# NethermindEth/stark-rings

Measured on AMD Instinct MI355X. Metric: ring-muls/sec (Goldilocks, deg 2^16, batch 2^14), higher is better.
Workload: dtype u64; 1 GPU; goldilocks_d65536_b16384; ring=goldilocks, degree=65536, batch_per_gpu=16384, global_batch=16384, layout=ark-ff Montgomery u64 limbs, in place (a *= b), b read-only, variant=mul, parallelism=batch-sharded x1, twiddle broadcast only

## Files before the change

include/stark_rings_hip.h:

```cpp
#ifndef STARK_RINGS_HIP_H
#define STARK_RINGS_HIP_H

#include <stddef.h>
#include <stdint.h>

#ifdef __cplusplus
extern "C" {
#endif

enum sr_ring {
    SR_RING_GOLDILOCKS_POW2 = 0,
    SR_RING_BABYBEAR_POW2 = 1,
    SR_RING_STARK_POW2 = 2,
    SR_RING_GOLDILOCKS_24 = 3,
    SR_RING_BABYBEAR_72 = 4,
    SR_RING_FROG_16 = 5
};

enum sr_status {
    SR_OK = 0,
    SR_E_INVALID = 1,
    SR_E_NO_DEVICE = 2,
    SR_E_HIP = 3,
    SR_E_ALLOC = 4,
    SR_E_UNSUPPORTED = 5
};

typedef struct sr_ctx sr_ctx;

int sr_ctx_create(int ring, int log2_degree, int device, sr_ctx **out);
enum sr_plan_flags {
    SR_PLAN_GENERIC_KERNELS = 1u << 0,
    SR_PLAN_GL_NO_COLS256 = 1u << 1,
    SR_PLAN_RT_NO_COLS256 = 1u << 2,
    SR_PLAN_GL_REGTILE = 1u << 3,
    SR_PLAN_STARK_NO_LAZY = 1u << 4,
    SR_PLAN_STARK_GENERIC_ON_LAZY = 1u << 5,
    SR_PLAN_NO_HOST_PIN = 1u << 6,
    SR_PLAN_GL_PLAIN_COLS = 1u << 7,
    SR_PLAN_GL_SPLIT_ROWS = 1u << 8
};
typedef struct sr_plan {
    uint32_t flags;
    int32_t log_tile;
    int32_t stark_whole_max;
    uint32_t chunk_polys;
    uint64_t scratch_limit_bytes;
    uint32_t host_chunk_mb;
    uint32_t lanes;
} sr_plan;
int sr_ctx_create_ex(int ring, int log2_degree, int device, const sr_plan *plan, sr_ctx **out);
int sr_ctx_reserve_scratch(sr_ctx *ctx, size_t batch);
int sr_ctx_plan_in_use(sr_ctx *ctx, sr_plan *plan, double probe_ms[2], size_t *probe_elems);
int sr_ctx_destroy(sr_ctx *ctx);
int sr_ctx_degree(const sr_ctx *ctx, size_t *degree);
int sr_ctx_limbs(const sr_ctx *ctx, int *limbs);
int sr_ctx_twiddle_block(sr_ctx *ctx, void **dev_ptr, size_t *bytes);
int sr_ctx_twiddles_updated(sr_ctx *ctx);
int sr_ctx_create_group(int ring, int log2_degree, const int *device_ids, int n, const sr_plan *plan, sr_ctx **out);
int sr_shard_range(size_t batch, int n, int i, size_t *first, size_t *count);

int sr_ntt_fwd_batch(sr_ctx *ctx, uint64_t *data, size_t batch);
int sr_ntt_inv_batch(sr_ctx *ctx, uint64_t *data, size_t batch);
int sr_pointwise_mul_batch(sr_ctx *ctx, uint64_t *lhs_inout, const uint64_t *rhs, size_t batch);
int sr_add_batch(sr_ctx *ctx, uint64_t *lhs_inout, const uint64_t *rhs, size_t batch);
int sr_sub_batch(sr_ctx *ctx, uint64_t *lhs_inout, const uint64_t *rhs, size_t batch);
int sr_neg_batch(sr_ctx *ctx, uint64_t *data, size_t batch);
int sr_scale_batch(sr_ctx *ctx, uint64_t *data, const uint64_t *scalar, size_t batch);
int sr_add_scalar_batch(sr_ctx *ctx, uint64_t *data, const uint64_t *scalar, int ntt_form, size_t batch);
int sr_mul_elem_batch(sr_ctx *ctx, uint64_t *data_inout, const uint64_t *elem, size_t batch);
int sr_sum_batch(sr_ctx *ctx, uint64_t *out, const uint64_t *in, size_t n);
int sr_product_batch(sr_ctx *ctx, uint64_t *out, const uint64_t *in_ntt, size_t n);
int sr_mul_elem_add_batch(sr_ctx *ctx, uint64_t *acc_inout, const uint64_t *x, const uint64_t *r, size_t batch);
int sr_ring_mul_batch(sr_ctx *ctx, uint64_t *out, const uint64_t *a, const uint64_t *b, size_t batch);
int sr_reduce_batch(sr_ctx *ctx, const uint64_t *in, size_t in_len_per_elem, uint64_t *out, size_t batch);

int sr_ntt_fwd_batch_dev(sr_ctx *ctx, uint64_t *d_data, size_t batch, void *stream);
int sr_ntt_inv_batch_dev(sr_ctx *ctx, uint64_t *d_data, size_t batch, void *stream);
int sr_pointwise_mul_batch_dev(sr_ctx *ctx, uint64_t *d_lhs_inout, const uint64_t *d_rhs, size_t batch, void *stream);
int sr_add_batch_dev(sr_ctx *ctx, uint64_t *d_lhs_inout, const uint64_t *d_rhs, size_t batch, void *stream);
int sr_sub_batch_dev(sr_ctx *ctx, uint64_t *d_lhs_inout, const uint64_t *d_rhs, size_t batch, void *stream);
int sr_neg_batch_dev(sr_ctx *ctx, uint64_t *d_data, size_t batch, void *stream);
int sr_scale_batch_dev(sr_ctx *ctx, uint64_t *d_data, const uint64_t *host_scalar, size_t batch, void *stream);
int sr_add_scalar_batch_dev(sr_ctx *ctx, uint64_t *d_data, const uint64_t *host_scalar, int ntt_form, size_t batch, void *stream);
int sr_mul_elem_batch_dev(sr_ctx *ctx, uint64_t *d_data_inout, const uint64_t *d_elem, size_t batch, void *stream);
int sr_sum_batch_dev(sr_ctx *ctx, uint64_t *d_out, const uint64_t *d_in, size_t n, void *stream);
int sr_product_batch_dev(sr_ctx *ctx, uint64_t *d_out, const uint64_t *d_in_ntt, size_t n, void *stream);
int sr_mul_elem_add_batch_dev(sr_ctx *ctx, uint64_t *d_acc_inout, const uint64_t *d_x, const uint64_t *d_r, size_t batch, void *stream);
enum { SR_MLE_LEADING = 0, SR_MLE_TRAILING = 1 };
int sr_mle_plan(int ring, int log2_degree, size_t num_vars, size_t n_fixed, int order, size_t *work_elems, int *launches);
int sr_mle_fix_variables_dev(sr_ctx *ctx, uint64_t *d_out, const uint64_t *d_evals, size_t n_evals, size_t num_vars, const uint64_t *d_point,
                             size_t n_fixed, int order, uint64_t *d_work, size_t work_elems, void *stream);
int sr_mle_fix_variables(sr_ctx *ctx, uint64_t *out, const uint64_t *evals, size_t n_evals, size_t num_vars, const uint64_t *point,
// ... 79 lines not shown
```

stark_rings_amd/_lib.py:

```python
import ctypes
import os

HERE = os.path.dirname(os.path.abspath(__file__))
LIB_PATH = os.environ.get("SR_LIB_PATH") or os.path.join(HERE, "libstarkrings_hip.so")

u64p = ctypes.POINTER(ctypes.c_uint64)
_c = ctypes

SYMBOLS = {
    "sr_ctx_create": (_c.c_int, [_c.c_int, _c.c_int, _c.c_int, _c.POINTER(_c.c_void_p)]),
    "sr_ctx_create_ex": (_c.c_int, [_c.c_int, _c.c_int, _c.c_int, _c.c_void_p, _c.POINTER(_c.c_void_p)]),
    "sr_ctx_create_group": (_c.c_int, [_c.c_int, _c.c_int, _c.POINTER(_c.c_int), _c.c_int, _c.c_void_p, _c.POINTER(_c.c_void_p)]),
    "sr_shard_range": (_c.c_int, [_c.c_size_t, _c.c_int, _c.c_int, _c.POINTER(_c.c_size_t), _c.POINTER(_c.c_size_t)]),
    "sr_ctx_reserve_scratch": (_c.c_int, [_c.c_void_p, _c.c_size_t]),
    "sr_ctx_plan_in_use": (_c.c_int, [_c.c_void_p, _c.c_void_p, _c.POINTER(_c.c_double), _c.POINTER(_c.c_size_t)]),
    "sr_ctx_destroy": (_c.c_int, [_c.c_void_p]),
    "sr_ctx_degree": (_c.c_int, [_c.c_void_p, _c.POINTER(_c.c_size_t)]),
    "sr_ctx_limbs": (_c.c_int, [_c.c_void_p, _c.POINTER(_c.c_int)]),
    "sr_ctx_twiddle_block": (_c.c_int, [_c.c_void_p, _c.POINTER(_c.c_void_p), _c.POINTER(_c.c_size_t)]),
    "sr_ctx_twiddles_updated": (_c.c_int, [_c.c_void_p]),
    "sr_ntt_fwd_batch": (_c.c_int, [_c.c_void_p, u64p, _c.c_size_t]),
    "sr_ntt_inv_batch": (_c.c_int, [_c.c_void_p, u64p, _c.c_size_t]),
    "sr_pointwise_mul_batch": (_c.c_int, [_c.c_void_p, u64p, u64p, _c.c_size_t]),
    "sr_add_batch": (_c.c_int, [_c.c_void_p, u64p, u64p, _c.c_size_t]),
# ... 36 lines not shown
    "sr_matmul_ntt": (_c.c_int, [_c.c_void_p] * 4 + [_c.c_size_t] * 3),
    "sr_decompose_balanced_batch_dev": (_c.c_int, [_c.c_void_p] * 3 + [_c.c_uint64, _c.c_size_t, _c.c_size_t, _c.c_void_p]),
    "sr_decompose_overflow_count": (_c.c_int, [_c.c_void_p, _c.POINTER(_c.c_ulonglong), _c.c_void_p]),
    "sr_recompose_batch_dev": (_c.c_int, [_c.c_void_p] * 3 + [_c.c_uint64, _c.c_size_t, _c.c_size_t, _c.c_void_p]),
    "sr_decompose_balanced_batch": (_c.c_int, [_c.c_void_p] * 3 + [_c.c_uint64, _c.c_size_t, _c.c_size_t]),
    "sr_recompose_batch": (_c.c_int, [_c.c_void_p] * 3 + [_c.c_uint64, _c.c_size_t, _c.c_size_t]),
    "sr_decompose_balanced_batch_wide_dev": (_c.c_int, [_c.c_void_p] * 3 + [_c.c_uint64, _c.c_uint64, _c.c_size_t, _c.c_size_t, _c.c_void_p]),
    "sr_recompose_batch_wide_dev": (_c.c_int, [_c.c_void_p] * 3 + [_c.c_uint64, _c.c_uint64, _c.c_size_t, _c.c_size_t, _c.c_void_p]),
    "sr_decompose_balanced_batch_wide": (_c.c_int, [_c.c_void_p] * 3 + [_c.c_uint64, _c.c_uint64, _c.c_size_t, _c.c_size_t]),
    "sr_recompose_batch_wide": (_c.c_int, [_c.c_void_p] * 3 + [_c.c_uint64, _c.c_uint64, _c.c_size_t, _c.c_size_t]),
    "sr_wire_coeff_bytes": (_c.c_size_t, [_c.c_void_p]),
    "sr_serialize_batch_dev": (_c.c_int, [_c.c_void_p] * 4 + [_c.c_size_t, _c.c_void_p]),
    "sr_deserialize_batch_dev": (_c.c_int, [_c.c_void_p] * 4 + [_c.c_size_t, _c.c_void_p]),
    "sr_wire_invalid_count": (_c.c_int, [_c.c_void_p, _c.POINTER(_c.c_ulonglong), _c.c_void_p]),
    "sr_serialize_batch": (_c.c_int, [_c.c_void_p] * 3 + [_c.c_size_t]),
    "sr_deserialize_batch": (_c.c_int, [_c.c_void_p] * 3 + [_c.c_size_t]),
    "sr_rot_batch_dev": (_c.c_int, [_c.c_void_p] * 3 + [_c.c_size_t, _c.c_void_p]),
    "sr_rot_batch": (_c.c_int, [_c.c_void_p, u64p, _c.c_size_t]),
    "sr_ring_mul_batch_dev": (_c.c_int, [_c.c_void_p, _c.c_void_p, _c.c_void_p, _c.c_void_p, _c.c_size_t, _c.c_void_p]),
    "sr_ring_mul_ntt_rhs_batch": (_c.c_int, [_c.c_void_p, u64p, u64p, u64p, _c.c_size_t]),
    "sr_ring_mul_ntt_rhs_batch_dev": (_c.c_int, [_c.c_void_p, _c.c_void_p, _c.c_void_p, _c.c_void_p, _c.c_size_t, _c.c_void_p]),
    "sr_pack32_batch_dev": (_c.c_int, [_c.c_void_p, _c.c_void_p, _c.c_void_p, _c.c_size_t, _c.c_void_p]),
    "sr_unpack32_batch_dev": (_c.c_int, [_c.c_void_p, _c.c_void_p, _c.c_void_p, _c.c_size_t, _c.c_void_p]),
    "sr_ntt_fwd_packed32_batch_dev": (_c.c_int, [_c.c_void_p, _c.c_void_p, _c.c_size_t, _c.c_void_p]),
    "sr_ntt_inv_packed32_batch_dev": (_c.c_int, [_c.c_void_p, _c.c_void_p, _c.c_size_t, _c.c_void_p]),
    "sr_ring_mul_packed32_batch_dev": (_c.c_int, [_c.c_void_p, _c.c_void_p, _c.c_void_p, _c.c_void_p, _c.c_size_t, _c.c_void_p]),
    "sr_pointwise_mul_packed32_batch_dev": (_c.c_int, [_c.c_void_p, _c.c_void_p, _c.c_void_p, _c.c_size_t, _c.c_void_p]),
    "sr_add_packed32_batch_dev": (_c.c_int, [_c.c_void_p, _c.c_void_p, _c.c_void_p, _c.c_size_t, _c.c_void_p]),
    "sr_sub_packed32_batch_dev": (_c.c_int, [_c.c_void_p, _c.c_void_p, _c.c_void_p, _c.c_size_t, _c.c_void_p]),
    "sr_reduce_batch_dev": (_c.c_int, [_c.c_void_p, _c.c_void_p, _c.c_size_t, _c.c_void_p, _c.c_size_t, _c.c_void_p]),
    "sr_fill_uniform_dev": (_c.c_int, [_c.c_void_p, _c.c_uint64, _c.c_uint64, _c.c_size_t, _c.c_void_p, _c.c_void_p]),
    "sr_count_noncanonical_dev": (_c.c_int, [_c.c_void_p, _c.c_void_p, _c.c_size_t, _c.POINTER(_c.c_uint64), _c.c_void_p]),
    "sr_ctx_profile_enable": (_c.c_int, [_c.c_void_p, _c.c_int]),
    "sr_ctx_profile_read": (_c.c_int, [_c.c_void_p, _c.POINTER(_c.c_double), _c.POINTER(_c.c_uint64)]),
    "sr_ctx_profile_read_sampled": (_c.c_int, [_c.c_void_p, _c.POINTER(_c.c_double), _c.POINTER(_c.c_uint64), _c.POINTER(_c.c_uint64)]),
    "sr_selftest_field_op": (_c.c_int, [_c.c_int, _c.c_int, u64p, u64p, u64p]),
    "sr_selftest_rep_counters": (_c.c_int, [u64p, _c.c_int]),
    "sr_last_error_string": (_c.c_char_p, []),
    "sr_version": (_c.c_char_p, []),
}



class Plan(ctypes.Structure):
    _fields_ = [("flags", _c.c_uint32), ("log_tile", _c.c_int32), ("stark_whole_max", _c.c_int32), ("chunk_polys", _c.c_uint32),
                ("scratch_limit_bytes", _c.c_uint64), ("host_chunk_mb", _c.c_uint32), ("lanes", _c.c_uint32)]


PLAN_GENERIC_KERNELS, PLAN_GL_NO_COLS256, PLAN_RT_NO_COLS256 = 1, 2, 4
PLAN_GL_REGTILE, PLAN_STARK_NO_LAZY, PLAN_STARK_GENERIC_ON_LAZY = 8, 16, 32
PLAN_NO_HOST_PIN = 64
PLAN_GL_PLAIN_COLS = 128
PLAN_GL_SPLIT_ROWS = 256


def plan_from_env(ring=None):
    e = os.environ
    f = 0
    if (ring in (None, 0) and e.get("SR_GOLDILOCKS_GENERIC") == "1") or (ring in (None, 1) and e.get("SR_BABYBEAR_GENERIC") == "1"):
        f |= PLAN_GENERIC_KERNELS
    if e.get("SR_GL_COLS256") == "0":
        f |= PLAN_GL_NO_COLS256
    if e.get("SR_RT_COLS256") == "0":
        f |= PLAN_RT_NO_COLS256
    if e.get("SR_GOLDILOCKS_REGTILE") == "1":
        f |= PLAN_GL_REGTILE
    if e.get("SR_STARK_LAZY") == "0":
        f |= PLAN_STARK_NO_LAZY
    if e.get("SR_STARK_TUNED") == "0":
        f |= PLAN_STARK_GENERIC_ON_LAZY
    if e.get("SR_HOST_PIN") == "0":
        f |= PLAN_NO_HOST_PIN
    if e.get("SR_GL_KEEP_COLS") == "0":
        f |= PLAN_GL_PLAIN_COLS
    if e.get("SR_GL_SPLIT_ROWS") == "1":
        f |= PLAN_GL_SPLIT_ROWS
    p = Plan()
    p.flags = f
    p.log_tile = int(e.get("SR_LOG_TILE", "0") or 0)
    p.stark_whole_max = int(e.get("SR_ST_WHOLE_MAX", "0") or 0)
    p.chunk_polys = int(e.get("SR_CHUNK_POLYS", "0") or 0)
    p.scratch_limit_bytes = int(e.get("SR_SCRATCH_LIMIT_MB", "0") or 0) << 20
    p.host_chunk_mb = int(e.get("SR_HOST_CHUNK_MB", "0") or 0)
    p.lanes = int(e.get("SR_LANES", "0") or 0)
    return p


_lib = None


class BackendMissing(RuntimeError):
    pass


def load():
    global _lib
    if _lib is None:
        if not os.path.exists(LIB_PATH):
            raise BackendMissing(
                "%s not found: run `python -c 'import __graft_entry__ as g; g.build()'` "
                "(hipcc --offload-arch=gfx950).  There is no CPU fallback." % LIB_PATH
            )
        try:
            import torch
        except Exception:
            pass
        lib = ctypes.CDLL(LIB_PATH)
        for name, (res, args) in SYMBOLS.items():
            fn = getattr(lib, name)
            fn.restype = res
            fn.argtypes = args
        _lib = lib
    return _lib


def last_error():
    return load().sr_last_error_string().decode()
```

stark_rings_amd/csrc/capi.hip:

```cpp
#include "../../include/stark_rings_hip.h"

#include <hip/hip_runtime.h>

#include <cstdio>
#include <cstring>
#include <condition_variable>
#include <functional>
#include <initializer_list>
#include <mutex>
#include <string>
#include <thread>
#include <type_traits>
#include <vector>

#include "fields.hpp"
#include "ntt_generic.hpp"
#include "ntt_goldilocks.hpp"
#include "ntt_regtile.hpp"
#include "small_rings.hpp"
#include "small_linalg.hpp"
#include "decompose.hpp"
#include "wire.hpp"
#include "frog_ring.hpp"
#include "ntt_stark.hpp"
// ... 248 lines not shown
    const int k = c->k;
    if (k > F::kTwoAdicity - 1) return fail(SR_E_INVALID, "log2_degree exceeds the field's 2-adicity");
    c->log_tile = default_log_tile<F>();
    if (c->plan.log_tile >= 8 && c->plan.log_tile <= 12) c->log_tile = c->plan.log_tile;
    if (k > 2 * c->log_tile && !stark_tuned) return fail(SR_E_INVALID, "log2_degree too large for the two-level kernels");
    const size_t d = c->degree;
    size_t extra = 0;
    if constexpr (std::is_same<F, sr::Goldilocks>::value) extra = sr::gl_fast_extra_bytes(k);
    c->table_bytes = 2 * d * sizeof(E) + extra;
    HIP_TRY(hipMalloc(&c->tables, c->table_bytes));

    uint64_t e[4];
    exponent_pm1_shift<F>(k + 1, e);
    E psi = sr::pow_tw<F>(F::tw_from_u64(F::kGenerator), e, 4);
    E psi_inv = inv_tw<F>(psi);
    std::vector<E> pows(k + 1), ipows(k + 1);
    pows[0] = psi;
    ipows[0] = psi_inv;
    for (int j = 1; j <= k; j++) {
        pows[j] = F::mul_tw(pows[j - 1], pows[j - 1]);
        ipows[j] = F::mul_tw(ipows[j - 1], ipows[j - 1]);
    }
    E *d_pows = nullptr;
    HIP_TRY(hipMalloc(&d_pows, 2 * (k + 1) * sizeof(E)));
    HIP_TRY(hipMemcpy(d_pows, pows.data(), (k + 1) * sizeof(E), hipMemcpyHostToDevice));
    HIP_TRY(hipMemcpy(d_pows + (k + 1), ipows.data(), (k + 1) * sizeof(E), hipMemcpyHostToDevice));
    E *tw = (E *)c->tables, *itw = tw + d;
    unsigned blocks = (unsigned)((d + 255) / 256);
    if (blocks > 4096) blocks = 4096;
    hipLaunchKernelGGL(sr::build_tables_kernel<F>, dim3(blocks), dim3(256), 0, c->stream, tw, itw, k, d_pows,
                       d_pows + (k + 1));
    HIP_TRY(hipGetLastError());
    HIP_TRY(hipStreamSynchronize(c->stream));
    HIP_TRY(hipFree(d_pows));

    E dinv = inv_tw<F>(F::tw_from_u64((uint64_t)d));
    E two = F::tw_from_u64(2);
    E kappa = pow_small<F>(two, kappa_bits<F>());
    E rb_inv = inv_tw<F>(pow_small<F>(two, F::kBoundaryBits));
    E fused = F::mul_tw(dinv, F::mul_tw(kappa, rb_inv));
    E half_turn_inv = k >= 1 ? ipows[k - 1] : F::tw_one();
    E s0 = sr::Lazy<F>::table(dinv), s1 = sr::Lazy<F>::table(F::mul_tw(dinv, half_turn_inv));
    E m0 = sr::Lazy<F>::table(fused), m1 = sr::Lazy<F>::table(F::mul_tw(fused, half_turn_inv));
    memcpy(c->inv_scale0, &s0, sizeof(E));
    memcpy(c->inv_scale1, &s1, sizeof(E));
    memcpy(c->mul_scale0, &m0, sizeof(E));
    memcpy(c->mul_scale1, &m1, sizeof(E));
    if constexpr (std::is_same<F, sr::Goldilocks>::value) {
        if (sr::gl_fast_init(c->gl_fast, k, (const uint64_t *)tw, (const uint64_t *)itw, (uint64_t *)(itw + d),
                             (const uint64_t *)pows.data(), (const uint64_t *)ipows.data(), (uint64_t)dinv,
                             (uint64_t)fused, !(c->plan.flags & SR_PLAN_GL_NO_COLS256), c->plan.chunk_polys, c->stream))
            return fail(SR_E_HIP, "goldilocks fast-path table build failed");
        c->gl_fast.keep_cols = !(c->plan.flags & SR_PLAN_GL_PLAIN_COLS);
        c->gl_fast.split_rows = (c->plan.flags & SR_PLAN_GL_SPLIT_ROWS) != 0 && k > 12;
    }
    return SR_OK;
}

template <class F>
sr::NttParams<F> make_params(const sr_ctx *c, bool fused) {
    using E = typename F::elem;
    sr::NttParams<F> p;
    p.k = c->k;
    p.log_tile = c->log_tile;
    p.s_rows = c->k > c->log_tile ? c->k - c->log_tile : 0;
    p.tw = (const E *)c->tables;
    p.itw = p.tw + c->degree;
    memcpy(&p.scale0, fused ? c->mul_scale0 : c->inv_scale0, sizeof(E));
    memcpy(&p.scale1, fused ? c->mul_scale1 : c->inv_scale1, sizeof(E));
    return p;
}

template <class F>
size_t lds_bytes(const sr_ctx *c, bool two_buffers) {
    return ((size_t)F::kLdsWords * 4u << c->log_tile) * (two_buffers ? 2 : 1);
}

template <class F, int MODE>
int launch_rows(sr_ctx *c, typename F::storage *a, const typename F::storage *b, typename F::storage *out,
                size_t batch, bool fused_scale, hipStream_t st) {
    const size_t n = batch << c->k;
    const size_t tiles = (n + ((size_t)1 << c->log_tile) - 1) >> c->log_tile;
    if (tiles > 0x7FFFFFFFull) return fail(SR_E_INVALID, "batch too large for one launch");
    auto p = make_params<F>(c, fused_scale);
    ProfScope ps(c, st, K_ROWS);
    hipLaunchKernelGGL((sr::rows_kernel<F, MODE>), dim3((unsigned)tiles), dim3(sr::kThreads),
                       lds_bytes<F>(c, MODE == sr::MODE_MUL), st, a, b, out, n, p);
    HIP_TRY(hipGetLastError());
    return SR_OK;
}
template <class F, int MODE>
int launch_cols(sr_ctx *c, typename F::storage *a, const typename F::storage *src, size_t batch, bool fused_scale, hipStream_t st) {
    const size_t blocks = batch << (c->k - c->log_tile);
    if (blocks > 0x7FFFFFFFull) return fail(SR_E_INVALID, "batch too large for one launch");
    auto p = make_params<F>(c, fused_scale);
    ProfScope ps(c, st, MODE == sr::MODE_FWD ? K_FWD_COLS : K_INV_COLS);
    hipLaunchKernelGGL((sr::cols_kernel<F, MODE>), dim3((unsigned)blocks), dim3(sr::kThreads), lds_bytes<F>(c, false),
                       st, a, src, batch, p);
    HIP_TRY(hipGetLastError());
    return SR_OK;
}

template <class F>
int fwd_dev(sr_ctx *c, uint64_t *d, size_t batch, hipStream_t st) {
    auto *a = reinterpret_cast<typename F::storage *>(d);
    if (c->k == 0 || batch == 0) return SR_OK;
// ... 2173 lines not shown
```

stark_rings_amd/csrc/ntt_goldilocks.hpp:

```cpp
#pragma once
#include <utility>

#include "fields.hpp"

namespace sr {
namespace gl {

using G = Goldilocks;
typedef uint64_t u64;
typedef uint32_t u32;

constexpr int kW16Exp = 156;

__device__ __forceinline__ u64 ld_stream(const u64 *p) { return __builtin_nontemporal_load(p); }
__device__ __forceinline__ void st_stream(u64 *p, u64 v) { __builtin_nontemporal_store(v, p); }
__device__ __forceinline__ u64 ld_scratch(const u64 *p) { return *p; }
__device__ __forceinline__ void st_scratch(u64 *p, u64 v) { *p = v; }
__device__ __forceinline__ void st_result(u64 *p, u64 v) {
    repcheck::leaves_library(v);
    st_stream(p, v);
}
__device__ __forceinline__ void st_slots(u64 *p, u64 v) {
    repcheck::leaves_library(v);
    *p = v;
// ... 497 lines not shown
        dft16_fwd_hot(x);
#pragma unroll
        for (int sg = 0; sg < 16; sg++)
            st_scratch(reinterpret_cast<u64 *>(pb + (offB + (unsigned)sg * leg)), G::mul(x[sg], tw[sg]));
    } else {
        u64 tw[16];
#pragma unroll
        for (int sg = 0; sg < 16; sg++) {
            x[sg] = ld_scratch(reinterpret_cast<const u64 *>(ps + (offB + (unsigned)sg * leg)));
            tw[sg] = *reinterpret_cast<const u64 *>(tb + (offB + (unsigned)sg * leg));
        }
#pragma unroll
        for (int sg = 0; sg < 16; sg++) x[sg] = G::mul(x[sg], tw[sg]);
        dft16_inv_hot(x);
#pragma unroll
        for (int j = 0; j < 16; j++) lds[CT::idx(16 * rg + j, col)] = x[j];
        __syncthreads();
#pragma unroll
        for (int h = 0; h < 16; h++) x[h] = lds[CT::idx(16 * h + rg, col)];
#pragma unroll
        for (int h = 0; h < 16; h++) x[h] = G::mul(x[h], wc[h * 16 + rg]);
        cols_stage_inv<3>(x);
        cols_stage_inv<2>(x);
        cols_stage_inv<1>(x);
        cols_stage_inv<0>(x);
#pragma unroll
        for (int jj = 0; jj < 16; jj++) st_result(reinterpret_cast<u64 *>(pb + (offA + (unsigned)jj * 16u * leg)), x[jj]);
    }
}

constexpr int kColsXcdGroup = 4;
template <int DIR, int LC>
__global__ __launch_bounds__(16 << LC, 4) void cols256_kernel(u64 *data, const u64 *src, int k, const u64 *__restrict__ wc,
                                                              const u64 *__restrict__ twist, unsigned grouped) {
    __shared__ u64 lds[ColsTile<LC>::kElems];
    __shared__ u64 wl[256];
    if (threadIdx.x < 256) wl[threadIdx.x] = wc[threadIdx.x];
    __syncthreads();
    cols256_tile<DIR, LC>(xcd_tile(blockIdx.x, kColsXcdGroup, grouped), data, src, k, wl, twist, lds);
}
template <int LC>
__global__ __launch_bounds__(16 << LC, 4) void cols256_pair_kernel(u64 *data_a, const u64 *src_a, u64 *data_b, const u64 *src_b, int k,
                                                                   const u64 *__restrict__ wc, const u64 *__restrict__ twist,
                                                                   unsigned grouped, unsigned tiles) {
    __shared__ u64 lds[ColsTile<LC>::kElems];
    __shared__ u64 wl[256];
    if (threadIdx.x < 256) wl[threadIdx.x] = wc[threadIdx.x];
    __syncthreads();
    const unsigned v = xcd_tile(blockIdx.x, kColsXcdGroup, grouped);
    const bool second = v >= tiles;
    cols256_tile<0, LC>(second ? v - tiles : v, second ? data_b : data_a, second ? src_b : src_a, k, wl, twist, lds);
}

template <int DIR>
__global__ __launch_bounds__(256, 3) void cols256_keep_kernel(u64 *data, const u64 *src, u64 *data2, const u64 *src2, int k,
                                                              const u64 *__restrict__ wc, const u64 *__restrict__ twist, unsigned npoly,
                                                              unsigned groups) {
    using CT = ColsTile<4>;
    __shared__ u64 lds[CT::kElems];
    __shared__ u64 wl[256];
    const int t = threadIdx.x;
    wl[t] = wc[t];
    const int ls = k - 8;
    const unsigned chunks = 1u << (ls - 4);
    const unsigned xcd = blockIdx.x & 7u, slot = blockIdx.x >> 3;
    const unsigned ci = slot & (chunks - 1u), grp = slot >> (ls - 4);
    const int col = t & 15, rg = t >> 4;
    const unsigned i = ci * 16u + (unsigned)col;
    const char *tb = reinterpret_cast<const char *>(twist);
    const unsigned leg = 8u << ls;
    const unsigned offA0 = (((unsigned)rg << ls) + i) * 8u;
    const unsigned offB0 = (((unsigned)rg << (ls + 4)) + i) * 8u;
    u64 x[16], tw[16];
#pragma unroll
    for (int sg = 0; sg < 16; sg++) tw[sg] = *reinterpret_cast<const u64 *>(tb + (offB0 + (unsigned)sg * leg));
    __syncthreads();
    const unsigned total = data2 ? 2u * npoly : npoly;
    for (unsigned it = xcd + 8u * grp; it < total; it += 8u * groups) {
        const bool second = it >= npoly;
        const unsigned poly = second ? it - npoly : it;
        char *pb = reinterpret_cast<char *>((second ? data2 : data) + ((size_t)poly << k));
        const char *ps = reinterpret_cast<const char *>((second ? src2 : src) + ((size_t)poly << k));
        unsigned offA = offA0, offB = offB0;
        asm volatile("" : "+v"(offA), "+v"(offB));
        if (DIR == 0) {
#pragma unroll
            for (int jj = 0; jj < 16; jj++) x[jj] = ld_stream(reinterpret_cast<const u64 *>(ps + (offA + (unsigned)jj * 16u * leg)));
            cols_stage_fwd<0>(x);
            cols_stage_fwd<1>(x);
            cols_stage_fwd<2>(x);
            cols_stage_fwd<3>(x);
#pragma unroll
            for (int h = 0; h < 16; h++) {
                x[h] = G::mul(x[h], wl[h * 16 + rg]);
                if ((h & 3) == 3) __builtin_amdgcn_sched_barrier(0);
            }
#pragma unroll
            for (int h = 0; h < 16; h++) lds[CT::idx(16 * h + rg, col)] = x[h];
            __syncthreads();
#pragma unroll
            for (int j = 0; j < 16; j++) x[j] = lds[CT::idx(16 * rg + j, col)];
            dft16_fwd_hot(x);
#pragma unroll
            for (int sg = 0; sg < 16; sg++) st_scratch(reinterpret_cast<u64 *>(pb + (offB + (unsigned)sg * leg)), G::mul(x[sg], tw[sg]));
        } else {
#pragma unroll
            for (int sg = 0; sg < 16; sg++) x[sg] = ld_scratch(reinterpret_cast<const u64 *>(ps + (offB + (unsigned)sg * leg)));
#pragma unroll
            for (int sg = 0; sg < 16; sg++) {
                x[sg] = G::mul(x[sg], tw[sg]);
                if ((sg & 3) == 3) __builtin_amdgcn_sched_barrier(0);
            }
            dft16_inv_hot(x);
#pragma unroll
            for (int j = 0; j < 16; j++) lds[CT::idx(16 * rg + j, col)] = x[j];
            __syncthreads();
#pragma unroll
            for (int h = 0; h < 16; h++) x[h] = lds[CT::idx(16 * h + rg, col)];
#pragma unroll
            for (int h = 0; h < 16; h++) {
                x[h] = G::mul(x[h], wl[h * 16 + rg]);
                if ((h & 3) == 3) __builtin_amdgcn_sched_barrier(0);
            }
            cols_stage_inv<3>(x);
            cols_stage_inv<2>(x);
            cols_stage_inv<1>(x);
            cols_stage_inv<0>(x);
#pragma unroll
            for (int jj = 0; jj < 16; jj++) st_result(reinterpret_cast<u64 *>(pb + (offA + (unsigned)jj * 16u * leg)), x[jj]);
        }
        __syncthreads();
    }
}

template <int Q, bool TW, int P = kPhased, bool CANON = false>
__device__ __forceinline__ void tile_fwd(const u64 *__restrict__ src, u64 *lds, const int t, const Tables &T, u64 *x,
                                         int nvalid) {
    constexpr bool LZ = !TW && Q == 0;
#pragma unroll
    for (int j = 0; j < 16; j++) {
        const int pos = j * 256 + t;
        x[j] = TW ? ld_stream(src + (pos < nvalid ? pos : nvalid - 1)) : ld_scratch(src + pos);
    }
    if (TW) twist_rows<Q, false>(x, std::make_integer_sequence<int, 16>{});
    if constexpr (LZ) dft16_fwd_dit<P, true>(x);
    else dft16_fwd_q<Q, P>(x);
    if (TW) x[0] = G::mul(x[0], T.w1f[t]);
#pragma unroll
    for (int r = 1; r < 16; r++) x[r] = G::mul(x[r], T.w1f[r * 256 + t]);
#pragma unroll
    for (int r = 0; r < 16; r++) lds[pad(r * 256 + t)] = x[r];
    __syncthreads();
    const int i0 = t & 15, base2 = (t >> 4) * 256 + i0;
#pragma unroll
    for (int j = 0; j < 16; j++) x[j] = lds[pad(base2 + j * 16)];
    if constexpr (LZ) dft16_fwd_dit<P, true>(x);
    else dft16_fwd<P>(x);
#pragma unroll
    for (int s = 1; s < 16; s++) x[s] = G::mul(x[s], T.w2f[s * 16 + i0]);
#pragma unroll
    for (int s = 0; s < 16; s++) lds[pad(base2 + s * 16)] = x[s];
    __syncthreads();
#pragma unroll
    for (int j = 0; j < 16; j++) x[j] = lds[17 * t + j];
    if constexpr (LZ) dft16_fwd_dit<P, !CANON>(x);
    else dft16_fwd<P>(x);
}

template <int Q, bool TW, int P = kPhased>
__device__ __forceinline__ void tile_inv(u64 *x, u64 *lds, const int t, const Tables &T, const u64 *w1i,
                                         u64 *__restrict__ dst, int nvalid) {
    constexpr bool LZ = !TW && Q == 0;
    dft16_inv<P, LZ>(x);
#pragma unroll
    for (int j = 0; j < 16; j++) lds[17 * t + j] = x[j];
    __syncthreads();
    const int i0 = t & 15, base2 = (t >> 4) * 256 + i0;
#pragma unroll
    for (int s = 0; s < 16; s++) x[s] = lds[pad(base2 + s * 16)];
#pragma unroll
    for (int s = 1; s < 16; s++) x[s] = G::mul(x[s], T.w2i[s * 16 + i0]);
    if (LZ) x[0] = G::canon(x[0]);
    dft16_inv<P, LZ>(x);
#pragma unroll
// ... 185 lines not shown


__device__ __forceinline__ u64 pow_from_bits(const u64 *pw, unsigned e, int k) {
    u64 acc = 1;
    for (int j = 0; j <= k; j++)
        if ((e >> j) & 1u) acc = G::mul(acc, pw[j]);
    return acc;
}
__global__ void build_tables_kernel(int k, int c, const u64 *pows, const u64 *ipows, u64 dinv, u64 dinv_mul, u64 *twist_f,
                                    u64 *twist_i_plain, u64 *twist_i_mul, u64 *w1f, u64 *w1i, u64 *w1i_mul, u64 *w2f,
                                    u64 *w2i, u64 *wcf, u64 *wci) {
    const int q = 12 - (k - c);
    const size_t d = (size_t)1 << k;
    const size_t n = d > 4096 ? d : 4096;
    const unsigned mask2d = (unsigned)(2 * d - 1);
    for (size_t idx = blockIdx.x * (size_t)blockDim.x + threadIdx.x; idx < n; idx += (size_t)gridDim.x * blockDim.x) {
        if (idx < d) {
            unsigned b = (unsigned)(idx >> (k - c)), i = (unsigned)(idx & ((d >> c) - 1));
            unsigned e = (unsigned)(((unsigned long long)(2 * bitrev(b, c) + 1) * i) & mask2d);
            twist_f[idx] = pow_from_bits(pows, e, k);
            u64 inv = pow_from_bits(ipows, e, k);
            twist_i_plain[idx] = G::mul(inv, dinv);
            twist_i_mul[idx] = G::mul(inv, dinv_mul);
        }
        if (idx < 4096) {
            unsigned r = (unsigned)(idx >> 8), i0 = (unsigned)(idx & 255);
            unsigned m0 = bitrev(r & ((1u << (4 - q)) - 1u), 4 - q);
            unsigned e1 = (unsigned)((((unsigned long long)i0 * m0) << (c + 1)) & mask2d);
            if (k <= 12) e1 = (e1 + i0) & mask2d;
            w1f[idx] = pow_from_bits(pows, e1, k);
            const u64 inv1 = pow_from_bits(ipows, e1, k);
            w1i[idx] = k <= 12 ? G::mul(inv1, dinv) : inv1;
            w1i_mul[idx] = k <= 12 ? G::mul(inv1, dinv_mul) : inv1;
        }
        if (idx < 256) {
            unsigned s = (unsigned)(idx >> 4), i0 = (unsigned)(idx & 15);
            unsigned e2 = (unsigned)((((unsigned long long)i0 * bitrev(s, 4)) << (k - 7)) & mask2d);
            w2f[idx] = pow_from_bits(pows, e2, k);
            w2i[idx] = pow_from_bits(ipows, e2, k);
            unsigned e3 = (unsigned)((((unsigned long long)(2 * bitrev(s, 4) + 1) * i0) << (k - 8)) & mask2d);
            wcf[idx] = pow_from_bits(pows, e3, k);
            wci[idx] = pow_from_bits(ipows, e3, k);
        }
    }
}

}

struct GoldilocksFastTables {
    int k = -1;
    int c = 0;
    bool cols256 = false;
    bool keep_cols = true;
    bool split_rows = false;
    bool ready = false;
    gl::Tables t{};
    size_t chunk_polys = 0;
    void (*prof_begin)(void *user, int tag, hipStream_t st) = nullptr;
    void (*prof_end)(void *user, hipStream_t st) = nullptr;
    void *prof_user = nullptr;
};
struct GlProfScope {
    const GoldilocksFastTables &f;
    hipStream_t st;
    GlProfScope(const GoldilocksFastTables &ff, int tag, hipStream_t s) : f(ff), st(s) {
        if (f.prof_begin) f.prof_begin(f.prof_user, tag, st);
    }
    ~GlProfScope() {
        if (f.prof_end) f.prof_end(f.prof_user, st);
    }
};

inline bool gl_fast_supported(const GoldilocksFastTables &f) { return f.ready; }
inline size_t gl_fast_extra_bytes(int k) {
    if (k < 8 || k > 22) return 0;
    return (((size_t)3 << k) + 3 * 4096 + 4 * 256) * sizeof(uint64_t);
}
inline int gl_fast_init(GoldilocksFastTables &f, int k, const uint64_t *tw, const uint64_t *itw, uint64_t *extra,
                        const uint64_t *host_pows, const uint64_t *host_ipows, uint64_t dinv, uint64_t dinv_mul,
                        bool allow_cols256, size_t chunk_polys, hipStream_t st) {
    f.k = k;
    f.ready = false;
    if (gl_fast_extra_bytes(k) == 0) return 0;
    const size_t d = (size_t)1 << k;
    uint64_t *p = extra;
    uint64_t *twist_f = p;            p += d;
    uint64_t *twist_ip = p;           p += d;
    uint64_t *twist_im = p;           p += d;
    uint64_t *w1f = p;                p += 4096;
    uint64_t *w1i = p;                p += 4096;
    uint64_t *w1im = p;               p += 4096;
    uint64_t *w2f = p;                p += 256;
    uint64_t *w2i = p;                p += 256;
    uint64_t *wcf = p;                p += 256;
    uint64_t *wci = p;
    f.cols256 = k >= 16 && k <= 20 && allow_cols256;
    f.chunk_polys = chunk_polys;
    f.c = f.cols256 ? 8 : (k > 12 ? k - 12 : 0);
    uint64_t *d_pows = nullptr;
    if (hipMalloc(&d_pows, 2 * (k + 1) * sizeof(uint64_t)) != hipSuccess) return 1;
    bool ok = hipMemcpy(d_pows, host_pows, (k + 1) * 8, hipMemcpyHostToDevice) == hipSuccess &&
              hipMemcpy(d_pows + k + 1, host_ipows, (k + 1) * 8, hipMemcpyHostToDevice) == hipSuccess;
    if (ok) {
        unsigned blocks = (unsigned)(((d > 4096 ? d : 4096) + 255) / 256);
        if (blocks > 4096) blocks = 4096;
        hipLaunchKernelGGL(gl::build_tables_kernel, dim3(blocks), dim3(256), 0, st, k, f.c, d_pows, d_pows + k + 1, dinv, dinv_mul,
// ... 21 lines not shown
        case 0: hipLaunchKernelGGL((gl::strided_kernel<0, DIR, TWIST>), g, b, 0, st, data, src, k, s_lo, tw, twist); break;
        case 1: hipLaunchKernelGGL((gl::strided_kernel<1, DIR, TWIST>), g, b, 0, st, data, src, k, s_lo, tw, twist); break;
        case 2: hipLaunchKernelGGL((gl::strided_kernel<2, DIR, TWIST>), g, b, 0, st, data, src, k, s_lo, tw, twist); break;
        case 3: hipLaunchKernelGGL((gl::strided_kernel<3, DIR, TWIST>), g, b, 0, st, data, src, k, s_lo, tw, twist); break;
        case 4: hipLaunchKernelGGL((gl::strided_kernel<4, DIR, TWIST>), g, b, 0, st, data, src, k, s_lo, tw, twist); break;
        default: return 1;
    }
    return hipGetLastError() != hipSuccess;
}
template <int DIR, bool TWIST>
inline int gl_launch_strided256(const GoldilocksFastTables &f, uint64_t *data, const uint64_t *src, int k, int s_lo, size_t npoly,
                                const uint64_t *tw, const uint64_t *twist, hipStream_t st) {
    GlProfScope ps(f, DIR == 0 ? 0 : 2, st);
    const size_t S = (size_t)1 << (k - s_lo - 8);
    const size_t blocks = npoly * ((size_t)1 << s_lo) * (S >> 4);
    if (blocks == 0 || blocks > 0x7FFFFFFFull) return 1;
    hipLaunchKernelGGL((gl::strided256_kernel<DIR, TWIST>), dim3((unsigned)blocks), dim3(256), 0, st, data, src, k, s_lo, tw,
                       twist);
    return hipGetLastError() != hipSuccess;
}
inline int gl_plan(int c, int *ms) {
    int n = 0;
    const bool big = c >= 8;
    if (big) c -= 8;
    while (c > 0) {
        int m = c > 4 ? (c + 1) / 2 : c;
        ms[n++] = m;
        c -= m;
    }
    if (big) ms[n++] = 8;
    return n;
}
template <int DIR>
inline int gl_launch_cols256(const GoldilocksFastTables &f, uint64_t *data, const uint64_t *src, size_t npoly,
                             const uint64_t *wc, const uint64_t *twist, hipStream_t st) {
    GlProfScope ps(f, DIR == 0 ? 0 : 2, st);
    constexpr int LC = 4;
    const size_t blocks = npoly << (f.k - 8 - LC);
    if (blocks == 0 || blocks > 0x7FFFFFFFull) return 1;
    const unsigned grouped = xcd_grouped_tiles(blocks, gl::kColsXcdGroup);
    hipLaunchKernelGGL((gl::cols256_kernel<DIR, LC>), dim3((unsigned)blocks), dim3(16 << LC), 0, st, data, src, f.k, wc, twist,
                       grouped);
    return hipGetLastError() != hipSuccess;
}
template <int DIR>
inline int gl_launch_cols256_lane(const GoldilocksFastTables &f, uint64_t *data, const uint64_t *src, size_t npoly, const uint64_t *wc,
                                  const uint64_t *twist, hipStream_t st) {
    const unsigned chunks = 1u << (f.k - 12);
    unsigned groups = chunks >= 128 ? 1u : 128u / chunks;
    if (!f.keep_cols || f.k != 16 || (npoly & 7u) != 0 || npoly < 16u || npoly > 0x7FFFFFFFull)
        return gl_launch_cols256<DIR>(f, data, src, npoly, wc, twist, st);
    if (groups > npoly / 16) groups = (unsigned)(npoly / 16);
    GlProfScope ps(f, DIR == 0 ? 0 : 2, st);
    hipLaunchKernelGGL((gl::cols256_keep_kernel<DIR>), dim3(8u * chunks * groups), dim3(256), 0, st, data, src, (uint64_t *)nullptr,
                       (const uint64_t *)nullptr, f.k, wc, twist, (unsigned)npoly, groups);
    return hipGetLastError() != hipSuccess;
}
inline int gl_launch_cols256_pair_plain(const GoldilocksFastTables &f, uint64_t *da, const uint64_t *sa, uint64_t *db, const uint64_t *sb,
                                        size_t npoly, hipStream_t st) {
    GlProfScope ps(f, 0, st);
    constexpr int LC = 4;
    const size_t blocks = npoly << (f.k - 8 - LC);
    if (blocks == 0 || blocks > 0x3FFFFFFFull) return 1;
    hipLaunchKernelGGL((gl::cols256_pair_kernel<LC>), dim3((unsigned)(2 * blocks)), dim3(16 << LC), 0, st, da, sa, db, sb, f.k, f.t.wcf,
                       f.t.twist_f, xcd_grouped_tiles(2 * blocks, gl::kColsXcdGroup), (unsigned)blocks);
    return hipGetLastError() != hipSuccess;
}
inline int gl_launch_cols256_lane_pair(const GoldilocksFastTables &f, uint64_t *da, const uint64_t *sa, uint64_t *db, const uint64_t *sb,
                                       size_t npoly, hipStream_t st) {
    const unsigned chunks = 1u << (f.k - 12);
    unsigned groups = chunks >= 128 ? 1u : 128u / chunks;
    if (!f.keep_cols || f.k != 16 || (npoly & 7u) != 0 || npoly < 16u || npoly > 0x3FFFFFFFull)
        return gl_launch_cols256_pair_plain(f, da, sa, db, sb, npoly, st);
    if (groups > npoly / 16) groups = (unsigned)(npoly / 16);
    GlProfScope ps(f, 0, st);
    hipLaunchKernelGGL((gl::cols256_keep_kernel<0>), dim3(8u * chunks * groups), dim3(256), 0, st, da, sa, db, sb, f.k, f.t.wcf, f.t.twist_f,
                       (unsigned)npoly, groups);
    return hipGetLastError() != hipSuccess;
}
inline int gl_strided_fwd(const GoldilocksFastTables &f, uint64_t *d, const uint64_t *src, size_t npoly, hipStream_t st) {
    if (f.cols256) return gl_launch_cols256<0>(f, d, src, npoly, f.t.wcf, f.t.twist_f, st);
    int ms[8];
    const int n = gl_plan(f.k > 12 ? f.k - 12 : 0, ms);
    int s_lo = 0;
    for (int p = 0; p < n; p++) {
        const bool last = p == n - 1;
        const uint64_t *from = p == 0 ? src : d;
        int rc;
        if (ms[p] == 8)
            rc = last ? gl_launch_strided256<0, true>(f, d, from, f.k, s_lo, npoly, f.t.tw, f.t.twist_f, st)
                      : gl_launch_strided256<0, false>(f, d, from, f.k, s_lo, npoly, f.t.tw, nullptr, st);
        else
            rc = last ? gl_launch_strided<0, true>(f, ms[p], d, from, f.k, s_lo, npoly, f.t.tw, f.t.twist_f, st)
                      : gl_launch_strided<0, false>(f, ms[p], d, from, f.k, s_lo, npoly, f.t.tw, nullptr, st);
        if (rc) return rc;
        s_lo += ms[p];
    }
    return 0;
}
inline int gl_strided_inv(const GoldilocksFastTables &f, uint64_t *d, size_t npoly, bool fused, hipStream_t st) {
    const uint64_t *tw_i = fused ? f.t.twist_i_mul : f.t.twist_i_plain;
    if (f.cols256) return gl_launch_cols256<1>(f, d, d, npoly, f.t.wci, tw_i, st);
    int ms[8];
    const int n = gl_plan(f.k > 12 ? f.k - 12 : 0, ms);
    int s_lo = f.k > 12 ? f.k - 12 : 0;
    for (int p = n - 1; p >= 0; p--) {
        s_lo -= ms[p];
        const bool first = p == n - 1;
        int rc;
        if (ms[p] == 8)
            rc = first ? gl_launch_strided256<1, true>(f, d, d, f.k, s_lo, npoly, f.t.itw, tw_i, st)
                       : gl_launch_strided256<1, false>(f, d, d, f.k, s_lo, npoly, f.t.itw, nullptr, st);
        else
            rc = first ? gl_launch_strided<1, true>(f, ms[p], d, d, f.k, s_lo, npoly, f.t.itw, tw_i, st)
                       : gl_launch_strided<1, false>(f, ms[p], d, d, f.k, s_lo, npoly, f.t.itw, nullptr, st);
        if (rc) return rc;
    }
    return 0;
}
template <int MODE>
inline int gl_launch_rows(const GoldilocksFastTables &f, uint64_t *a, const uint64_t *b, uint64_t *out, size_t npoly,
                          bool fused, hipStream_t st) {
    const size_t n_total = npoly << f.k;
    const size_t tiles = (n_total + gl::kTile - 1) / gl::kTile;
    if (tiles == 0 || tiles > 0x7FFFFFFFull) return 1;
    GlProfScope ps(f, 1, st);
    const uint64_t *w1i = fused ? f.t.w1i_mul : f.t.w1i;
    dim3 g((unsigned)tiles), blk(256);
#define SR_GL_ROWS(QQ, TT) hipLaunchKernelGGL((gl::rows_kernel<MODE, QQ, TT>), g, blk, 0, st, a, b, out, f.t, w1i, n_total)
    const bool tw = f.c == 0;
// ... 114 lines not shown
```

Baseline: 1.144 million ring-muls/s.

## Prefetch next polynomial into LDS via global_load_lds in keep-cols kernel

Adds a DMA variant of the persistent cols256 keep kernel. It uses global_load_lds to asynchronously fetch the next polynomial's column tile directly into LDS while the current one is being transformed. The transpose exchange moves to a padded (stride 17) LDS layout, and the end-of-iteration syncthreads is replaced by finer lgkmcnt/vmcnt barriers. The intent is to hide global load latency behind compute. The cost is extra LDS traffic, a reused LDS buffer with subtle ordering hazards, and possible bank-conflict or occupancy changes. The variant is on by default and can be disabled with SR_GL_KEEP_DMA=0.

```diff
diff --git a/include/stark_rings_hip.h b/include/stark_rings_hip.h
--- a/include/stark_rings_hip.h
+++ b/include/stark_rings_hip.h
@@ -38,7 +38,8 @@
     SR_PLAN_STARK_GENERIC_ON_LAZY = 1u << 5,
     SR_PLAN_NO_HOST_PIN = 1u << 6,
     SR_PLAN_GL_PLAIN_COLS = 1u << 7,
-    SR_PLAN_GL_SPLIT_ROWS = 1u << 8
+    SR_PLAN_GL_SPLIT_ROWS = 1u << 8,
+    SR_PLAN_GL_KEEP_NO_DMA = 1u << 9
 };
 typedef struct sr_plan {
     uint32_t flags;
diff --git a/stark_rings_amd/_lib.py b/stark_rings_amd/_lib.py
--- a/stark_rings_amd/_lib.py
+++ b/stark_rings_amd/_lib.py
@@ -112,6 +112,7 @@
 PLAN_NO_HOST_PIN = 64
 PLAN_GL_PLAIN_COLS = 128
 PLAN_GL_SPLIT_ROWS = 256
+PLAN_GL_KEEP_NO_DMA = 512
 
 
 def plan_from_env(ring=None):
@@ -135,6 +136,8 @@
         f |= PLAN_GL_PLAIN_COLS
     if e.get("SR_GL_SPLIT_ROWS") == "1":
         f |= PLAN_GL_SPLIT_ROWS
+    if e.get("SR_GL_KEEP_DMA") == "0":
+        f |= PLAN_GL_KEEP_NO_DMA
     p = Plan()
     p.flags = f
     p.log_tile = int(e.get("SR_LOG_TILE", "0") or 0)
diff --git a/stark_rings_amd/csrc/capi.hip b/stark_rings_amd/csrc/capi.hip
--- a/stark_rings_amd/csrc/capi.hip
+++ b/stark_rings_amd/csrc/capi.hip
@@ -324,6 +324,7 @@
                              (uint64_t)fused, !(c->plan.flags & SR_PLAN_GL_NO_COLS256), c->plan.chunk_polys, c->stream))
             return fail(SR_E_HIP, "goldilocks fast-path table build failed");
         c->gl_fast.keep_cols = !(c->plan.flags & SR_PLAN_GL_PLAIN_COLS);
+        c->gl_fast.keep_dma = !(c->plan.flags & SR_PLAN_GL_KEEP_NO_DMA);
         c->gl_fast.split_rows = (c->plan.flags & SR_PLAN_GL_SPLIT_ROWS) != 0 && k > 12;
     }
     return SR_OK;
diff --git a/stark_rings_amd/csrc/ntt_goldilocks.hpp b/stark_rings_amd/csrc/ntt_goldilocks.hpp
--- a/stark_rings_amd/csrc/ntt_goldilocks.hpp
+++ b/stark_rings_amd/csrc/ntt_goldilocks.hpp
@@ -573,7 +573,16 @@
     cols256_tile<0, LC>(second ? v - tiles : v, second ? data_b : data_a, second ? src_b : src_a, k, wl, twist, lds);
 }
 
-template <int DIR>
+template <bool NT>
+__device__ __forceinline__ void ld_lds16(const char *g, u64 *l) {
+    __builtin_amdgcn_global_load_lds((const __attribute__((address_space(1))) void *)g, (__attribute__((address_space(3))) void *)l, 16, 0,
+                                     NT ? 2 : 0);
+}
+__device__ __forceinline__ void lds_barrier() {
+    asm volatile("s_waitcnt lgkmcnt(0)" ::: "memory");
+    __builtin_amdgcn_s_barrier();
+}
+template <int DIR, bool DMA = false>
 __global__ __launch_bounds__(256, 3) void cols256_keep_kernel(u64 *data, const u64 *src, u64 *data2, const u64 *src2, int k,
                                                               const u64 *__restrict__ wc, const u64 *__restrict__ twist, unsigned npoly,
                                                               unsigned groups) {
@@ -597,16 +606,43 @@
     for (int sg = 0; sg < 16; sg++) tw[sg] = *reinterpret_cast<const u64 *>(tb + (offB0 + (unsigned)sg * leg));
     __syncthreads();
     const unsigned total = data2 ? 2u * npoly : npoly;
-    for (unsigned it = xcd + 8u * grp; it < total; it += 8u * groups) {
+    const unsigned step = 8u * groups;
+    const unsigned wv = __builtin_amdgcn_readfirstlane((unsigned)t >> 6), ln = (unsigned)t & 63u;
+    const unsigned dleg = DIR == 0 ? 64u * wv + (ln >> 3) : 16u * (ln >> 3) + 4u * wv;
+    const unsigned offD0 = ((dleg << ls) + ci * 16u) * 8u + (ln & 7u) * 16u;
+    auto fetch = [&](unsigned itn) {
+        const char *pn = reinterpret_cast<const char *>((itn >= npoly ? src2 : src) + ((size_t)(itn >= npoly ? itn - npoly : itn) << k));
+        unsigned offD = offD0;
+        asm volatile("" : "+v"(offD));
+#pragma unroll
+        for (unsigned q = 0; q < 8; q++)
+            ld_lds16<DIR == 0>(pn + (size_t)((DIR == 0 ? 8u * q : 128u * (q & 1u) + (q >> 1)) * leg) + offD, lds + (64u * wv + 8u * q) * 16u);
+    };
+    auto exchange_sync = [&]() {
+        if (DMA) lds_barrier();
+        else __syncthreads();
+    };
+    unsigned it = xcd + 8u * grp;
+    if (DMA && it < total) fetch(it);
+    for (; it < total; it += step) {
         const bool second = it >= npoly;
         const unsigned poly = second ? it - npoly : it;
         char *pb = reinterpret_cast<char *>((second ? data2 : data) + ((size_t)poly << k));
         const char *ps = reinterpret_cast<const char *>((second ? src2 : src) + ((size_t)poly << k));
         unsigned offA = offA0, offB = offB0;
         asm volatile("" : "+v"(offA), "+v"(offB));
+        if (DMA) {
+            asm volatile("s_waitcnt vmcnt(0)" ::: "memory");
+            __builtin_amdgcn_s_barrier();
+#pragma unroll
+            for (int j = 0; j < 16; j++) x[j] = lds[(rg + 16 * j) * 16 + col];
+            lds_barrier();
+        }
         if (DIR == 0) {
-#pragma unroll
-            for (int jj = 0; jj < 16; jj++) x[jj] = ld_stream(reinterpret_cast<const u64 *>(ps + (offA + (unsigned)jj * 16u * leg)));
+            if (!DMA) {
+#pragma unroll
+                for (int jj = 0; jj < 16; jj++) x[jj] = ld_stream(reinterpret_cast<const u64 *>(ps + (offA + (unsigned)jj * 16u * leg)));
+            }
             cols_stage_fwd<0>(x);
             cols_stage_fwd<1>(x);
             cols_stage_fwd<2>(x);
@@ -617,16 +653,22 @@
                 if ((h & 3) == 3) __builtin_amdgcn_sched_barrier(0);
             }
 #pragma unroll
-            for (int h = 0; h < 16; h++) lds[CT::idx(16 * h + rg, col)] = x[h];
-            __syncthreads();
-#pragma unroll
-            for (int j = 0; j < 16; j++) x[j] = lds[CT::idx(16 * rg + j, col)];
+            for (int h = 0; h < 16; h++) lds[DMA ? (16 * h + rg) * 17 + col : CT::idx(16 * h + rg, col)] = x[h];
+            exchange_sync();
+#pragma unroll
+            for (int j = 0; j < 16; j++) x[j] = lds[DMA ? (16 * rg + j) * 17 + col : CT::idx(16 * rg + j, col)];
+            if (DMA) {
+                lds_barrier();
+                if (it + step < total) fetch(it + step);
+            }
             dft16_fwd_hot(x);
 #pragma unroll
             for (int sg = 0; sg < 16; sg++) st_scratch(reinterpret_cast<u64 *>(pb + (offB + (unsigned)sg * leg)), G::mul(x[sg], tw[sg]));
         } else {
-#pragma unroll
-            for (int sg = 0; sg < 16; sg++) x[sg] = ld_scratch(reinterpret_cast<const u64 *>(ps + (offB + (unsigned)sg * leg)));
+            if (!DMA) {
+#pragma unroll
+                for (int sg = 0; sg < 16; sg++) x[sg] = ld_scratch(reinterpret_cast<const u64 *>(ps + (offB + (unsigned)sg * leg)));
+            }
 #pragma unroll
             for (int sg = 0; sg < 16; sg++) {
                 x[sg] = G::mul(x[sg], tw[sg]);
@@ -634,10 +676,14 @@
             }
             dft16_inv_hot(x);
 #pragma unroll
-            for (int j = 0; j < 16; j++) lds[CT::idx(16 * rg + j, col)] = x[j];
-            __syncthreads();
-#pragma unroll
-            for (int h = 0; h < 16; h++) x[h] = lds[CT::idx(16 * h + rg, col)];
+            for (int j = 0; j < 16; j++) lds[DMA ? (16 * rg + j) * 17 + col : CT::idx(16 * rg + j, col)] = x[j];
+            exchange_sync();
+#pragma unroll
+            for (int h = 0; h < 16; h++) x[h] = lds[DMA ? (16 * h + rg) * 17 + col : CT::idx(16 * h + rg, col)];
+            if (DMA) {
+                lds_barrier();
+                if (it + step < total) fetch(it + step);
+            }
 #pragma unroll
             for (int h = 0; h < 16; h++) {
                 x[h] = G::mul(x[h], wl[h * 16 + rg]);
@@ -650,7 +696,7 @@
 #pragma unroll
             for (int jj = 0; jj < 16; jj++) st_result(reinterpret_cast<u64 *>(pb + (offA + (unsigned)jj * 16u * leg)), x[jj]);
         }
-        __syncthreads();
+        if (!DMA) __syncthreads();
     }
 }
 
@@ -942,6 +988,7 @@
     int c = 0;
     bool cols256 = false;
     bool keep_cols = true;
+    bool keep_dma = true;
     bool split_rows = false;
     bool ready = false;
     gl::Tables t{};
@@ -1069,8 +1116,9 @@
         return gl_launch_cols256<DIR>(f, data, src, npoly, wc, twist, st);
     if (groups > npoly / 16) groups = (unsigned)(npoly / 16);
     GlProfScope ps(f, DIR == 0 ? 0 : 2, st);
-    hipLaunchKernelGGL((gl::cols256_keep_kernel<DIR>), dim3(8u * chunks * groups), dim3(256), 0, st, data, src, (uint64_t *)nullptr,
-                       (const uint64_t *)nullptr, f.k, wc, twist, (unsigned)npoly, groups);
+    const auto kernel = f.keep_dma ? gl::cols256_keep_kernel<DIR, true> : gl::cols256_keep_kernel<DIR, false>;
+    hipLaunchKernelGGL(kernel, dim3(8u * chunks * groups), dim3(256), 0, st, data, src, (uint64_t *)nullptr, (const uint64_t *)nullptr, f.k,
+                       wc, twist, (unsigned)npoly, groups);
     return hipGetLastError() != hipSuccess;
 }
 inline int gl_launch_cols256_pair_plain(const GoldilocksFastTables &f, uint64_t *da, const uint64_t *sa, uint64_t *db, const uint64_t *sb,
@@ -1091,8 +1139,9 @@
         return gl_launch_cols256_pair_plain(f, da, sa, db, sb, npoly, st);
     if (groups > npoly / 16) groups = (unsigned)(npoly / 16);
     GlProfScope ps(f, 0, st);
-    hipLaunchKernelGGL((gl::cols256_keep_kernel<0>), dim3(8u * chunks * groups), dim3(256), 0, st, da, sa, db, sb, f.k, f.t.wcf, f.t.twist_f,
-                       (unsigned)npoly, groups);
+    const auto kernel = f.keep_dma ? gl::cols256_keep_kernel<0, true> : gl::cols256_keep_kernel<0, false>;
+    hipLaunchKernelGGL(kernel, dim3(8u * chunks * groups), dim3(256), 0, st, da, sa, db, sb, f.k, f.t.wcf, f.t.twist_f, (unsigned)npoly,
+                       groups);
     return hipGetLastError() != hipSuccess;
 }
 inline int gl_strided_fwd(const GoldilocksFastTables &f, uint64_t *d, const uint64_t *src, size_t npoly, hipStream_t st) {
```

After: 1.140 million ring-muls/s. About the same (-0.4%).
